# Biogod2020/Spatial-Clip

Hardware: AMD Instinct MI355X
Metric: tile-gene pairs/sec (train step) (higher is better)
Workload: dtype bf16

## Files before the change

spatial-clip_amd/csrc/sc_gemm8p.hip:

```cpp
#include "sc_gemm_common.h"
#include <stdlib.h>
#include <map>
#include <mutex>

namespace {

constexpr int BM = 256, BN = 256, BK = 64;
constexpr int HALF = 128 * 64 * 2;
constexpr int RING = 8 * HALF;
constexpr int EPI_BYTES = 8 * 64 * SC_EPI_LD * 4;
constexpr int LDS_BYTES = EPI_BYTES > RING ? EPI_BYTES : RING;

typedef const __attribute__((address_space(1))) void* gptr_t;
typedef __attribute__((address_space(3))) void* lptr_t;

SC_DEVICE void dma16(const void* src, char* lds_wave_base) {
    __builtin_amdgcn_global_load_lds((gptr_t)src, (lptr_t)lds_wave_base, 16, 0, 0);
}

template <int EPI, bool Q8 = false, bool LUT = false, int NI = 8>
SC_DEVICE void epilogue_bf16_lds(f32x4 (&acc)[NI][4], const GemmArgs& g, char* strip, int row0, int col0, int lane,
                                 const unsigned* lut = nullptr) {
    float amax_lane = 0.f;
    const float q8s = (Q8 && sc_epi_gelu_fwd(EPI) && g.q8) ? *g.q8_scale : 0.f;
    const int li = lane & 15, lg = lane >> 4;
    constexpr bool kBias = (EPI == SC_EPI_BF16_BIAS || sc_epi_gelu_fwd(EPI));
    f32x4 bj[4];
#pragma unroll
    for (int j = 0; j < 4; ++j) {
        bj[j] = (f32x4){0.f, 0.f, 0.f, 0.f};
        const int c = col0 + j * 16 + lg * 4;
        if (kBias && g.bias && c < g.N) bj[j] = *reinterpret_cast<const f32x4*>(g.bias + c);
    }
    bf16* C = reinterpret_cast<bf16*>(g.C);
    bf16* C2 = reinterpret_cast<bf16*>(g.C2);
    const int rr = lane >> 3, rc = lane & 7;
    const int gcol = col0 + rc * 8;
#pragma unroll
    for (int p = 0; p < NI / 2; ++p) {
#pragma unroll
        for (int ib = 0; ib < 2; ++ib) {
            const int r = ib * 16 + li;
#pragma unroll
            for (int j = 0; j < 4; ++j) {
// ... 49 lines not shown
                            for (int e = 0; e < 8; ++e) {
                                float hv, gv;
                                sc_act_both((float)x.h[e], g.act, hv, gv);
                                o[e] = (bf16)hv;
                                gd[e] = (bf16)gv;
                            }
                        }
                        *reinterpret_cast<bf16x8*>(C + (size_t)grow * g.ldc + gcol) = gd;
                    }
                    *reinterpret_cast<bf16x8*>(C2 + (size_t)grow * g.ldc2 + gcol) = o;
                    if (Q8 && g.q8) {
                        float r[8];
#pragma unroll
                        for (int e = 0; e < 8; ++e) { r[e] = (float)o[e]; amax_lane = fmaxf(amax_lane, fabsf(r[e])); }
                        *reinterpret_cast<u32x2*>(g.q8 + (size_t)grow * g.ldq8 + gcol) = sc_pack8_fp8(r, q8s);
                    }
                }
            }
        }
        __builtin_amdgcn_s_waitcnt(0xC07F);
        __builtin_amdgcn_wave_barrier();
    }
    if (Q8 && sc_epi_gelu_fwd(EPI) && g.q8) sc_amax_publish(amax_lane, g.q8_amax);
}

constexpr int slot(int D, int q) { return D * 4 * HALF + q * HALF; }

struct Stager {
    const bf16* src[4][2];
    int nt;
    int wave;
};

template <int D, int PH>
SC_DEVICE void phase(char* smem, const Stager& S, int t, const int (&a_off)[2], const int (&b_off)[2], bf16x8 (&a)[8],
                     bf16x8 (&b0)[4], bf16x8 (&b1)[4], f32x4 (&acc)[8][4]) {
    if (PH == 1) {
#pragma unroll
        for (int kk = 0; kk < 2; ++kk)
#pragma unroll
            for (int jj = 0; jj < 2; ++jj)
                b0[kk * 2 + jj] = *reinterpret_cast<const bf16x8*>(smem + slot(D, 1) + b_off[kk] + jj * 2048);
    }
    if (PH == 2) {
#pragma unroll
        for (int kk = 0; kk < 2; ++kk)
#pragma unroll
            for (int jj = 0; jj < 2; ++jj)
                b1[kk * 2 + jj] = *reinterpret_cast<const bf16x8*>(smem + slot(D, 2) + b_off[kk] + jj * 2048);
    }
    if (PH == 1 || PH == 3) {
        constexpr int sl = slot(D, PH == 1 ? 0 : 3);
#pragma unroll
        for (int kk = 0; kk < 2; ++kk)
#pragma unroll
            for (int ii = 0; ii < 4; ++ii)
                a[kk * 4 + ii] = *reinterpret_cast<const bf16x8*>(smem + sl + a_off[kk] + ii * 2048);
    }
    constexpr int q = (PH + 1) & 3;
    constexpr int DS = PH <= 2 ? (D ^ 1) : D;
    const int ts = t + (PH <= 2 ? 1 : 2);
    if (ts < S.nt) {
        dma16(S.src[q][0] + (size_t)ts * BK, smem + slot(DS, q) + S.wave * 1024);
        dma16(S.src[q][1] + (size_t)ts * BK, smem + slot(DS, q) + (8 + S.wave) * 1024);
        asm volatile("s_waitcnt vmcnt(8)" ::: "memory");
    } else {
        asm volatile("s_waitcnt vmcnt(0)" ::: "memory");
    }
    __builtin_amdgcn_sched_barrier(0);
    __builtin_amdgcn_s_barrier();
    __builtin_amdgcn_sched_barrier(0);
    constexpr int mi = PH >= 3 ? 1 : 0;
    constexpr int nj = (PH == 2 || PH == 3) ? 1 : 0;
    __builtin_amdgcn_s_setprio(1);
#pragma unroll
    for (int kk = 0; kk < 2; ++kk)
#pragma unroll
        for (int ii = 0; ii < 4; ++ii)
#pragma unroll
            for (int jj = 0; jj < 2; ++jj)
                acc[mi * 4 + ii][nj * 2 + jj] =
                    sc_mfma16(nj ? b1[kk * 2 + jj] : b0[kk * 2 + jj], a[kk * 4 + ii], acc[mi * 4 + ii][nj * 2 + jj]);
    __builtin_amdgcn_s_setprio(0);
    __builtin_amdgcn_sched_barrier(0);
    __builtin_amdgcn_s_barrier();
    __builtin_amdgcn_sched_barrier(0);
}

template <int D>
SC_DEVICE void ktile(char* smem, const Stager& S, int t, const int (&a_off)[2], const int (&b_off)[2], bf16x8 (&a)[8],
                     bf16x8 (&b0)[4], bf16x8 (&b1)[4], f32x4 (&acc)[8][4]) {
    phase<D, 1>(smem, S, t, a_off, b_off, a, b0, b1, acc);
    phase<D, 2>(smem, S, t, a_off, b_off, a, b0, b1, acc);
    phase<D, 3>(smem, S, t, a_off, b_off, a, b0, b1, acc);
    phase<D, 4>(smem, S, t, a_off, b_off, a, b0, b1, acc);
}

constexpr int HRING = 9 * HALF;
constexpr int hslot(int D, int q) { return (D * 3 + q) * HALF; }

struct HStager {
    const bf16* src[3][2];
    int nt;
    int wave;
};

template <int D, int PH>
SC_DEVICE void hphase(char* smem, const HStager& S, int t, const int (&a_off)[2], const int (&b_off)[2], bf16x8 (&a)[8],
                      bf16x8 (&b0)[4], bf16x8 (&b1)[4], f32x4 (&acc)[4][4]) {
    if (PH == 1) {
#pragma unroll
        for (int kk = 0; kk < 2; ++kk)
#pragma unroll
            for (int jj = 0; jj < 2; ++jj)
                b0[kk * 2 + jj] = *reinterpret_cast<const bf16x8*>(smem + hslot(D, 1) + b_off[kk] + jj * 2048);
#pragma unroll
        for (int kk = 0; kk < 2; ++kk)
#pragma unroll
            for (int ii = 0; ii < 4; ++ii)
                a[kk * 4 + ii] = *reinterpret_cast<const bf16x8*>(smem + hslot(D, 0) + a_off[kk] + ii * 2048);
    } else {
#pragma unroll
        for (int kk = 0; kk < 2; ++kk)
#pragma unroll
            for (int jj = 0; jj < 2; ++jj)
                b1[kk * 2 + jj] = *reinterpret_cast<const bf16x8*>(smem + hslot(D, 2) + b_off[kk] + jj * 2048);
    }
    constexpr int DS = (D + 2) % 3;
    const int ts = t + 2;
    if (ts < S.nt) {
        if (PH == 1) {
            dma16(S.src[0][0] + (size_t)ts * BK, smem + hslot(DS, 0) + S.wave * 1024);
            dma16(S.src[0][1] + (size_t)ts * BK, smem + hslot(DS, 0) + (8 + S.wave) * 1024);
            dma16(S.src[1][0] + (size_t)ts * BK, smem + hslot(DS, 1) + S.wave * 1024);
            dma16(S.src[1][1] + (size_t)ts * BK, smem + hslot(DS, 1) + (8 + S.wave) * 1024);
            asm volatile("s_waitcnt vmcnt(10)" ::: "memory");
        } else {
            dma16(S.src[2][0] + (size_t)ts * BK, smem + hslot(DS, 2) + S.wave * 1024);
            dma16(S.src[2][1] + (size_t)ts * BK, smem + hslot(DS, 2) + (8 + S.wave) * 1024);
            asm volatile("s_waitcnt vmcnt(8)" ::: "memory");
        }
    } else {
        asm volatile("s_waitcnt vmcnt(0)" ::: "memory");
    }
    __builtin_amdgcn_sched_barrier(0);
    __builtin_amdgcn_s_barrier();
    __builtin_amdgcn_sched_barrier(0);
    constexpr int nj = PH - 1;
    __builtin_amdgcn_s_setprio(1);
#pragma unroll
    for (int kk = 0; kk < 2; ++kk)
#pragma unroll
        for (int ii = 0; ii < 4; ++ii)
#pragma unroll
            for (int jj = 0; jj < 2; ++jj)
                acc[ii][nj * 2 + jj] = sc_mfma16(nj ? b1[kk * 2 + jj] : b0[kk * 2 + jj], a[kk * 4 + ii], acc[ii][nj * 2 + jj]);
    __builtin_amdgcn_s_setprio(0);
    __builtin_amdgcn_sched_barrier(0);
    __builtin_amdgcn_s_barrier();
    __builtin_amdgcn_sched_barrier(0);
}

template <int D>
SC_DEVICE void hktile(char* smem, const HStager& S, int t, const int (&a_off)[2], const int (&b_off)[2], bf16x8 (&a)[8],
                      bf16x8 (&b0)[4], bf16x8 (&b1)[4], f32x4 (&acc)[4][4]) {
    hphase<D, 1>(smem, S, t, a_off, b_off, a, b0, b1, acc);
    hphase<D, 2>(smem, S, t, a_off, b_off, a, b0, b1, acc);
}

template <int EPI>
SC_DEVICE void half_tile(const GemmArgs& g, char* smem, int mh, int n0) {
    const int t = threadIdx.x;
    const int lane = t & 63;
    const int wave = __builtin_amdgcn_readfirstlane(t >> 6);
    const int wr = wave >> 2, wc = wave & 3;
    const int li = lane & 15, lg = lane >> 4;

    HStager S;
    S.nt = g.K / BK;
    S.wave = wave;
#pragma unroll
    for (int p = 0; p < 2; ++p) {
        const int r = (p * 8 + wave) * 8 + (lane >> 3);
        const int lc = (lane & 7) ^ ((r >> 1) & 7);
        const int ga = min(mh + r, g.M - 1);
        S.src[0][p] = g.A + (size_t)ga * g.lda + lc * 8;
#pragma unroll
        for (int h = 0; h < 2; ++h) {
            const int gb = min(n0 + (r >> 5) * 64 + h * 32 + (r & 31), g.N - 1);
            S.src[1 + h][p] = g.B + (size_t)gb * g.ldb + lc * 8;
        }
    }
    int a_off[2], b_off[2];
#pragma unroll
    for (int kk = 0; kk < 2; ++kk) {
        const int coff = ((kk * 4 + lg) ^ ((li >> 1) & 7)) << 4;
        a_off[kk] = (wr * 64 + li) * 128 + coff;
        b_off[kk] = (wc * 32 + li) * 128 + coff;
    }
    f32x4 acc[4][4];
#pragma unroll
    for (int i = 0; i < 4; ++i)
#pragma unroll
        for (int j = 0; j < 4; ++j) acc[i][j] = (f32x4){0.f, 0.f, 0.f, 0.f};

#pragma unroll
    for (int s = 0; s < 6; ++s) {
        const int ts = s / 3, q = s % 3;
        if (ts < S.nt) {
            dma16(S.src[q][0] + (size_t)ts * BK, smem + hslot(ts, q) + wave * 1024);
            dma16(S.src[q][1] + (size_t)ts * BK, smem + hslot(ts, q) + (8 + wave) * 1024);
        }
    }
    if (S.nt > 1) asm volatile("s_waitcnt vmcnt(8)" ::: "memory");
    else asm volatile("s_waitcnt vmcnt(0)" ::: "memory");
    __builtin_amdgcn_sched_barrier(0);
    __builtin_amdgcn_s_barrier();
    if (wr == 1) __builtin_amdgcn_s_barrier();
    __builtin_amdgcn_sched_barrier(0);

    bf16x8 a[8], b0[4], b1[4];
    for (int kt = 0; kt < S.nt; kt += 3) {
        hktile<0>(smem, S, kt, a_off, b_off, a, b0, b1, acc);
        if (kt + 1 < S.nt) hktile<1>(smem, S, kt + 1, a_off, b_off, a, b0, b1, acc);
        if (kt + 2 < S.nt) hktile<2>(smem, S, kt + 2, a_off, b_off, a, b0, b1, acc);
    }
    if (wr == 0) __builtin_amdgcn_s_barrier();
    asm volatile("s_waitcnt vmcnt(0)" ::: "memory");
    __builtin_amdgcn_sched_barrier(0);

    const int row0 = mh + wr * 64, col0 = n0 + wc * 64;
    if (EPI == SC_EPI_GELU_GRAD_PAIR && g.gelu_lut != nullptr) {
        unsigned* lut = reinterpret_cast<unsigned*>(smem + 8 * 4096);
        for (int c = t; c < SC_GELU_LUT_N / 4; c += 512)
            reinterpret_cast<u32x4*>(lut)[c] = reinterpret_cast<const u32x4*>(g.gelu_lut)[c];
        __syncthreads();
        epilogue_bf16_lds<EPI, false, true>(acc, g, smem + wave * 4096, row0, col0, lane, lut);
    } else if (EPI == SC_EPI_BF16 || EPI == SC_EPI_BF16_BIAS || sc_epi_gelu_fwd(EPI)) {
        epilogue_bf16_lds<EPI>(acc, g, smem + wave * 4096, row0, col0, lane);
    } else {
        float* ep = reinterpret_cast<float*>(smem) + wave * 64 * SC_EPI_LD;
        EpiRegs<EPI> er;
        sc_epi_load<EPI>(er, row0, col0, lane, g, 64);
#pragma unroll
        for (int i = 0; i < 4; ++i)
#pragma unroll
            for (int j = 0; j < 4; ++j) sc_epi_put(ep, i, j, li, lg, acc[i][j]);
        __builtin_amdgcn_s_waitcnt(0xC07F);
        __builtin_amdgcn_wave_barrier();
        sc_epilogue_store<EPI>(ep, er, row0, col0, lane, g, 0, -1, 64);
    }
}

template <int EPI>
__global__ __launch_bounds__(512, 2) void gemm8p_kernel(const GemmArgs g) {
    extern __shared__ __attribute__((aligned(16))) char smem[];
    int idx, hh = -1;
    if (g.tail_first > 0) {
        const int b = (int)blockIdx.x - g.tail_first;
        if (b >= 0) {
            const int r = sc_xcd_remap(b, 2 * g.tail_rem);
            idx = g.tail_first + (r >> 1);
            hh = r & 1;
        } else {
            idx = sc_xcd_remap(blockIdx.x, g.tail_first);
        }
    } else {
        idx = sc_xcd_remap(blockIdx.x, gridDim.x);
    }
    int tn, tm, z;
    if (g.col_group > 0) {
        sc_tile_colgroup(idx, g, tm, tn);
        z = 0;
    } else {
        tn = idx % g.ntn;
        idx /= g.ntn;
// ... 14 lines not shown
    const int m0 = tm * BM, n0 = tn * BN;
    const int kbeg = z * g.k_per_split;
    const int kend = min(g.K, kbeg + g.k_per_split);

    Stager S;
    S.nt = (kend - kbeg) / BK;
    S.wave = wave;
#pragma unroll
    for (int p = 0; p < 2; ++p) {
        const int r = (p * 8 + wave) * 8 + (lane >> 3);
        const int lc = (lane & 7) ^ ((r >> 1) & 7);
#pragma unroll
        for (int h = 0; h < 2; ++h) {
            const int ga = min(m0 + (r >> 6) * 128 + h * 64 + (r & 63), g.M - 1);
            const int gb = min(n0 + (r >> 5) * 64 + h * 32 + (r & 31), g.N - 1);
            S.src[h ? 3 : 0][p] = g.A + (size_t)ga * g.lda + kbeg + lc * 8;
            S.src[h ? 2 : 1][p] = g.B + (size_t)gb * g.ldb + kbeg + lc * 8;
        }
    }
    int a_off[2], b_off[2];
#pragma unroll
    for (int kk = 0; kk < 2; ++kk) {
        const int coff = ((kk * 4 + lg) ^ ((li >> 1) & 7)) << 4;
        a_off[kk] = (wr * 64 + li) * 128 + coff;
        b_off[kk] = (wc * 32 + li) * 128 + coff;
    }

    f32x4 acc[8][4];
#pragma unroll
    for (int i = 0; i < 8; ++i)
#pragma unroll
        for (int j = 0; j < 4; ++j) acc[i][j] = (f32x4){0.f, 0.f, 0.f, 0.f};

#pragma unroll
    for (int s = 0; s < 6; ++s) {
        const int ts = s >> 2, q = s & 3;
        if (ts < S.nt) {
            dma16(S.src[q][0] + (size_t)ts * BK, smem + slot(ts & 1, q) + wave * 1024);
            dma16(S.src[q][1] + (size_t)ts * BK, smem + slot(ts & 1, q) + (8 + wave) * 1024);
        }
    }
    if (S.nt > 1) asm volatile("s_waitcnt vmcnt(8)" ::: "memory");
    else asm volatile("s_waitcnt vmcnt(0)" ::: "memory");
    __builtin_amdgcn_sched_barrier(0);
    __builtin_amdgcn_s_barrier();
    if (wr == 1) __builtin_amdgcn_s_barrier();
    __builtin_amdgcn_sched_barrier(0);

    bf16x8 a[8], b0[4], b1[4];
    for (int kt = 0; kt < S.nt; kt += 2) {
        ktile<0>(smem, S, kt, a_off, b_off, a, b0, b1, acc);
        if (kt + 1 < S.nt) ktile<1>(smem, S, kt + 1, a_off, b_off, a, b0, b1, acc);
    }
    if (wr == 0) __builtin_amdgcn_s_barrier();
    asm volatile("s_waitcnt vmcnt(0)" ::: "memory");
    __builtin_amdgcn_sched_barrier(0);

    if (EPI == SC_EPI_GELU_GRAD_PAIR && g.gelu_lut != nullptr) {
        unsigned* lut = reinterpret_cast<unsigned*>(smem + 8 * 4096);
        for (int c = t; c < SC_GELU_LUT_N / 4; c += 512)
            reinterpret_cast<u32x4*>(lut)[c] = reinterpret_cast<const u32x4*>(g.gelu_lut)[c];
        __syncthreads();
        epilogue_bf16_lds<EPI, false, true>(acc, g, smem + wave * 4096, m0 + wr * 128, n0 + wc * 64, lane, lut);
    } else if (EPI == SC_EPI_BF16 || EPI == SC_EPI_BF16_BIAS || sc_epi_gelu_fwd(EPI)) {
        epilogue_bf16_lds<EPI>(acc, g, smem + wave * 4096, m0 + wr * 128, n0 + wc * 64, lane);
    } else {
        const int mw = wr * 128;
        float* ep = reinterpret_cast<float*>(smem) + wave * 64 * SC_EPI_LD;
        EpiRegs<EPI> er;
        sc_epi_load<EPI>(er, m0 + mw, n0 + wc * 64, lane, g, 64);
#pragma unroll
        for (int h = 0; h < 2; ++h) {
#pragma unroll
            for (int i = 0; i < 4; ++i)
#pragma unroll
                for (int j = 0; j < 4; ++j) sc_epi_put(ep, i, j, li, lg, acc[h * 4 + i][j]);
            __builtin_amdgcn_s_waitcnt(0xC07F);
            __builtin_amdgcn_wave_barrier();
            sc_epilogue_store<EPI>(ep, er, m0 + mw + h * 64, n0 + wc * 64, lane, g, z, (h + 1 < 2) ? m0 + mw + 64 : -1, 64);
            __builtin_amdgcn_s_waitcnt(0xC07F);
            __builtin_amdgcn_wave_barrier();
        }
    }
}

__global__ void sc_gelu_lut_fill_kernel(unsigned* lut, int act) {
    const int i = blockIdx.x * blockDim.x + threadIdx.x;
    if (i >= SC_GELU_LUT_N) return;
    const unsigned bits = (unsigned)(SC_GELU_LUT_LO + i % SC_GELU_LUT_HALF) | (i >= SC_GELU_LUT_HALF ? 0x8000u : 0u);
    const float u = __uint_as_float(bits << 16);
    float hv, gv;
    sc_act_both(u, act, hv, gv);
    union { bf16 b; unsigned short s; } h, gq;
    h.b = (bf16)hv;
    gq.b = (bf16)gv;
    lut[i] = ((unsigned)gq.s << 16) | (unsigned)h.s;
}

template <int EPI>
int launch(const GemmArgs& g, int nblocks, hipStream_t st) {
    static bool attr_done = false;
    if (!attr_done) {
        (void)hipFuncSetAttribute(reinterpret_cast<const void*>(&gemm8p_kernel<EPI>),
                                  hipFuncAttributeMaxDynamicSharedMemorySize, LDS_BYTES > HRING ? LDS_BYTES : HRING);
        attr_done = true;
    }
    const int lds = (g.tail_first > 0 && HRING > LDS_BYTES) ? HRING : LDS_BYTES;
    gemm8p_kernel<EPI><<<nblocks, 512, lds, st>>>(g);
    SC_LAUNCH_CHECK();
    return 1;
}


enum { PW_STEADY = 0, PW_POSTEPI = 1, PW_DRAIN0 = 2 };

struct PStager {
    const bf16* src[4][2];
    long long koff;
    int sk;
    int stile;
    int nt, wave, total, stride;
};

SC_DEVICE void pstage_set_tile(PStager& S, const GemmArgs& g, int lane) {
    const int tn = S.stile % g.ntn, tm = S.stile / g.ntn;
    const int m0 = tm * BM, n0 = tn * BN;
#pragma unroll
    for (int p = 0; p < 2; ++p) {
        const int r = (p * 8 + S.wave) * 8 + (lane >> 3);
        const int lc = (lane & 7) ^ ((r >> 1) & 7);
#pragma unroll
        for (int h = 0; h < 2; ++h) {
            const int ga = min(m0 + (r >> 6) * 128 + h * 64 + (r & 63), g.M - 1);
            const int gb = min(n0 + (r >> 5) * 64 + h * 32 + (r & 31), g.N - 1);
            S.src[h ? 3 : 0][p] = g.A + (size_t)ga * g.lda + lc * 8;
            S.src[h ? 2 : 1][p] = g.B + (size_t)gb * g.ldb + lc * 8;
        }
    }
}
SC_DEVICE void pstage_advance(PStager& S, const GemmArgs& g, int lane) {
// ... 918 lines not shown
    static bool attr_done = false;
    if (!attr_done) {
        (void)hipFuncSetAttribute(reinterpret_cast<const void*>(&gemm8p_tn_f8_kernel), hipFuncAttributeMaxDynamicSharedMemorySize,
                                  LDS_BYTES);
        attr_done = true;
    }
    sc_gemm_note_path(SC_GEMM_PATH_FP8_TN, 0, 0, splitk, g.colsum ? SC_GEMM_COLSUM_FUSED : SC_GEMM_COLSUM_NONE);
    gemm8p_tn_f8_kernel<<<g.ntm * g.ntn * splitk, 512, LDS_BYTES, st>>>(g);
    SC_LAUNCH_CHECK();
    return 1;
}

static int sc_colgroup_default(int epi, const GemmArgs& g) {
    (void)epi; (void)g;
    return 0;
}

extern "C" int sc_debug_gemm_tail_rule(int T, int S, int* nfull, int* rem) {
    const int r = (S > 0 && T > S) ? T % S : 0;
    const bool split = r > 0 && 2 * r <= S;
    if (nfull) *nfull = split ? T - r : T;
    if (rem) *rem = split ? r : 0;
    return split ? 1 : 0;
}

static int sc_last_tail[2] = {-1, -1};
extern "C" int sc_debug_gemm_last_tail(int* nfull, int* rem, int reset) {
    if (nfull) *nfull = sc_last_tail[0];
    if (rem) *rem = sc_last_tail[1];
    if (reset) sc_last_tail[0] = sc_last_tail[1] = -1;
    return 0;
}

static int sc_last_path[6] = {SC_GEMM_PATH_NONE, 0, 0, 0, SC_GEMM_COLSUM_NONE, SC_GEMM_GROUP_NONE};
void sc_gemm_note_path(int path, int lut, int col_group, int splitk, int colsum) {
    sc_last_path[0] = path; sc_last_path[1] = lut; sc_last_path[2] = col_group; sc_last_path[3] = splitk;
    sc_last_path[4] = colsum; sc_last_path[5] = SC_GEMM_GROUP_NONE;
}
void sc_gemm_note_colsum(int colsum) { sc_last_path[4] = colsum; }
void sc_gemm_note_group(int group) { sc_last_path[5] = group; }
extern "C" int sc_debug_gemm_last_path(int* out, int n, int reset) {
    for (int i = 0; i < n && i < 6; ++i) out[i] = sc_last_path[i];
    if (reset) sc_gemm_note_path(SC_GEMM_PATH_NONE, 0, 0, 0, SC_GEMM_COLSUM_NONE);
    return 6;
}

static int sc_gemm_slots() {
    static int cus[64] = {};
    int dev = 0;
    if (hipGetDevice(&dev) != hipSuccess || dev < 0 || dev >= 64) return 0;
    if (cus[dev] == 0) {
        int n = 0;
        if (hipDeviceGetAttribute(&n, hipDeviceAttributeMultiprocessorCount, dev) != hipSuccess || n < 1) n = -1;
        cus[dev] = n;
    }
    return cus[dev] > 0 ? cus[dev] : 0;
}

static bool sc_tail_default(int epi, const GemmArgs& g) {
    (void)epi; (void)g;
    return true;
}

int sc_gemm8p_try(int mode, int epi, GemmArgs& g, int splitk_req, float* slabs, hipStream_t st) {
    if (g.M < 256 || g.N < 192 || (g.K % BK) != 0) return 0;
    if (mode == SC_GEMM_TN && (epi != SC_EPI_F32 || (g.M % 8) != 0 || (g.N % 8) != 0)) return 0;
    if ((long long)g.M * g.N < 256LL * 256 * 8) return 0;
    if (mode == SC_GEMM_NT && splitk_req <= 1) {
        static const int small_tiles = getenv("SC_GEMM_SMALL_TILES") ? atoi(getenv("SC_GEMM_SMALL_TILES")) : 100;
        if ((long long)g.M * g.N < 256LL * 256 * small_tiles) return 0;
    }
    g.ntm = (g.M + BM - 1) / BM;
    g.ntn = (g.N + BN - 1) / BN;
    const int ktiles = g.K / BK;
    int splitk = splitk_req < 1 ? 1 : splitk_req;
    if (epi != SC_EPI_F32 || slabs == nullptr) splitk = 1;
    if (splitk > ktiles) splitk = ktiles;
    int tiles_per = (ktiles + splitk - 1) / splitk;
    splitk = (ktiles + tiles_per - 1) / tiles_per;
    g.splitk = splitk;
    g.k_per_split = tiles_per * BK;
    g.slab_stride = 0;
    if (splitk > 1) {
        if (g.ldc != g.N) return 0;
        g.C = slabs;
        g.slab_stride = (long long)g.M * g.N;
    }
    const int nblocks = g.ntm * g.ntn * splitk;
    if (mode == SC_GEMM_TN) {
        sc_gemm_note_path(SC_GEMM_PATH_TN8P, 0, 0, splitk, g.colsum ? SC_GEMM_COLSUM_FUSED : SC_GEMM_COLSUM_NONE);
        return launch_tn(g, nblocks, st);
    }
// ... 13 lines not shown
    g.col_group = 0;
    if (splitk == 1 && g.ntn > 1) {
        int gc = sc_colgroup_default(epi, g);
        if (const char* sw = getenv("SC_GEMM_COLGROUP")) {
            for (const char* p = sw; *p;) {
                char* e = nullptr;
                const long ep = strtol(p, &e, 10);
                if (e == p || *e != ':') break;
                const long v = strtol(e + 1, &e, 10);
                if (ep == epi || ep == -1) gc = (int)v;
                p = (*e == ',') ? e + 1 : e;
                if (*e != ',') break;
            }
        }
        if (gc > 0 && gc < g.ntn) {
            g.col_group = gc;
            g.band_rows = (g.ntm + 7) / 8;
        }
    }
    g.tail_first = g.tail_rem = 0;
    int grid = nblocks;
    if (splitk == 1) {
        const char* sw = getenv("SC_GEMM_TAIL");
        const int slots = sw ? atoi(sw) : (sc_tail_default(epi, g) ? sc_gemm_slots() : 0);
        int nfull = 0, rem = 0;
        if (slots > 0 && sc_debug_gemm_tail_rule(nblocks, slots, &nfull, &rem)) {
            g.tail_first = nfull;
            g.tail_rem = rem;
            grid = nfull + 2 * rem;
        }
    }
    sc_last_tail[0] = g.tail_first > 0 ? g.tail_first : nblocks;
    sc_last_tail[1] = g.tail_rem;
    sc_gemm_note_path(SC_GEMM_PATH_NT8P, g.gelu_lut != nullptr, g.col_group, splitk, SC_GEMM_COLSUM_NONE);
    int rc = 0;
#define SC_CASE(EPI) \
    if (epi == EPI) rc = launch<EPI>(g, grid, st);
    SC_CASE(SC_EPI_BF16)
    SC_CASE(SC_EPI_BF16_BIAS)
    SC_CASE(SC_EPI_F32_BIAS_RES)
    SC_CASE(SC_EPI_GELU_PAIR)
    SC_CASE(SC_EPI_BF16_DGELU)
    SC_CASE(SC_EPI_F32)
    SC_CASE(SC_EPI_BF16_BIAS_RES)
    SC_CASE(SC_EPI_GELU_GRAD_PAIR)
    SC_CASE(SC_EPI_BF16_MUL_AUX)
#undef SC_CASE
    return rc;
}

const unsigned* sc_gelu_lut_device(hipStream_t st, int act) {
    static std::mutex mu;
    static std::map<int, unsigned*> all;
    int dev = 0;
    if (hipGetDevice(&dev) != hipSuccess) return nullptr;
    const int key = dev * 2 + (act ? 1 : 0);
    std::lock_guard<std::mutex> lock(mu);
    auto it = all.find(key);
    if (it != all.end()) return it->second;
    unsigned* p = nullptr;
    if (hipMalloc(reinterpret_cast<void**>(&p), SC_GELU_LUT_N * sizeof(unsigned)) != hipSuccess) p = nullptr;
    if (p) {
        sc_gelu_lut_fill_kernel<<<(SC_GELU_LUT_N + 255) / 256, 256, 0, st>>>(p, act ? 1 : 0);
        if (hipGetLastError() != hipSuccess || hipStreamSynchronize(st) != hipSuccess) {
            (void)hipFree(p);
            p = nullptr;
        }
// ... 5 lines not shown
```

spatial-clip_amd/csrc/sc_gemm_common.h:

```cpp
#pragma once
#include "sc_common.h"
#include "sc_kernels.h"

struct GemmArgs {
    const bf16* A;
    const bf16* B;
    int M, N, K;
    int lda, ldb;
    void* C;
    int ldc;
    void* C2;
    int ldc2;
    const float* bias;
    const float* res;
    int ldres;
    const bf16* aux;
    int ldaux;
    int splitk;
    int k_per_split;
    long long slab_stride;
    int ntm, ntn;
    int tile_offset;
    float* colsum;
    const float* a_scale = nullptr;
    const float* b_scale = nullptr;
    unsigned char* q8 = nullptr;
    long long ldq8 = 0;
    const float* q8_scale = nullptr;
    float* q8_amax = nullptr;
    int a_scale_scalar = 0;
    const unsigned* gelu_lut = nullptr;
    int act = 0;
    int col_group = 0;
    int band_rows = 0;
    int tail_first = 0;
    int tail_rem = 0;
};

SC_DEVICE void sc_tile_colgroup(int idx, const GemmArgs& g, int& tm, int& tn) {
    const int band_tiles = g.band_rows * g.ntn;
    const int band = idx / band_tiles;
    const int r = idx - band * band_tiles;
    const int row0 = band * g.band_rows;
    const int rows = min(g.band_rows, g.ntm - row0);
    const int nfg = g.ntn / g.col_group;
    const int full = rows * g.col_group * nfg;
    if (r < full) {
        const int gsz = rows * g.col_group;
        const int grp = r / gsz, rr = r - grp * gsz;
        tm = row0 + rr / g.col_group;
        tn = grp * g.col_group + rr % g.col_group;
    } else {
        const int rem = g.ntn - nfg * g.col_group, r2 = r - full;
        tm = row0 + r2 / rem;
        tn = nfg * g.col_group + r2 % rem;
    }
}

constexpr int SC_GELU_LUT_LO = 107 << 7;
constexpr int SC_GELU_LUT_HALF = 25 * 128;
constexpr int SC_GELU_LUT_N = 2 * SC_GELU_LUT_HALF;
const unsigned* sc_gelu_lut_device(hipStream_t st, int act = 0);

constexpr int SC_EPI_LD = 68;

SC_DEVICE void sc_gelu_qe(float x, float& q, float& e) {
    const float y = fabsf(x) * 0.84932180028801904f;
    const float t = __builtin_amdgcn_rcpf(__builtin_fmaf(0.2727374808792225f, y, 1.0f));
    e = __builtin_amdgcn_exp2f(-(y * y));
// ... 50 lines not shown
constexpr bool sc_epi_gelu_fwd(int e) { return e == SC_EPI_GELU_PAIR || e == SC_EPI_GELU_GRAD_PAIR; }
constexpr bool sc_epi_aux_mul(int e) { return e == SC_EPI_BF16_DGELU || e == SC_EPI_BF16_MUL_AUX; }

SC_DEVICE u32x2 sc_pack8_fp8(const float (&v)[8], float s) {
    float c[8];
#pragma unroll
    for (int k = 0; k < 8; ++k) c[k] = fminf(fmaxf(v[k] * s, -448.f), 448.f);
    int w0 = __builtin_amdgcn_cvt_pk_fp8_f32(c[0], c[1], 0, false);
    w0 = __builtin_amdgcn_cvt_pk_fp8_f32(c[2], c[3], w0, true);
    int w1 = __builtin_amdgcn_cvt_pk_fp8_f32(c[4], c[5], 0, false);
    w1 = __builtin_amdgcn_cvt_pk_fp8_f32(c[6], c[7], w1, true);
    return (u32x2){(unsigned)w0, (unsigned)w1};
}
SC_DEVICE void sc_amax_publish(float amax_lane, float* slots) {
    float a = amax_lane;
#pragma unroll
    for (int off = 32; off > 0; off >>= 1) a = fmaxf(a, __shfl_xor(a, off, 64));
    if ((threadIdx.x & 63) == 0 && a > 0.f)
        atomicMax(reinterpret_cast<unsigned*>(slots) + (blockIdx.x & 63), __float_as_uint(a));
}

SC_DEVICE void sc_epi_put(float* ep, int row16, int col16, int li, int lg, f32x4 acc) {
    *reinterpret_cast<f32x4*>(ep + (row16 * 16 + li) * SC_EPI_LD + col16 * 16 + lg * 4) = acc;
}

template <int EPI>
struct EpiRegs {
    static constexpr bool kRes = (EPI == SC_EPI_F32_BIAS_RES);
    static constexpr bool kAux = (sc_epi_aux_mul(EPI) || EPI == SC_EPI_BF16_BIAS_RES);
    f32x4 r[kRes ? 16 : 1];
    bf16x8 a[kAux ? 8 : 1];
};

template <int EPI>
SC_DEVICE void sc_epi_load(EpiRegs<EPI>& e, int gm0, int gn0, int lane, const GemmArgs& g, int mrows = 64) {
    const int mlim = min(g.M, gm0 + mrows);
    if (EPI == SC_EPI_F32_BIAS_RES) {
        const int gn = gn0 + (lane & 15) * 4;
#pragma unroll
        for (int ps = 0; ps < 16; ++ps) {
            const int gm = gm0 + ps * 4 + (lane >> 4);
            e.r[ps] = (f32x4){0.f, 0.f, 0.f, 0.f};
            if (g.res && gm < mlim && gn < g.N) e.r[ps] = *reinterpret_cast<const f32x4*>(g.res + (size_t)gm * g.ldres + gn);
        }
    }
    if (sc_epi_aux_mul(EPI)) {
        const int gn = gn0 + (lane & 7) * 8;
#pragma unroll
        for (int ps = 0; ps < 8; ++ps) {
            const int gm = gm0 + ps * 8 + (lane >> 3);
            if (gm < mlim && gn < g.N) e.a[ps] = *reinterpret_cast<const bf16x8*>(g.aux + (size_t)gm * g.ldaux + gn);
        }
    }
    if (EPI == SC_EPI_BF16_BIAS_RES) {
        const int gn = gn0 + (lane & 7) * 8;
        const bf16* res = reinterpret_cast<const bf16*>(g.res);
#pragma unroll
        for (int ps = 0; ps < 8; ++ps) {
            const int gm = gm0 + ps * 8 + (lane >> 3);
#pragma unroll
            for (int k = 0; k < 8; ++k) e.a[ps][k] = (bf16)0.0f;
            if (res && gm < mlim && gn < g.N) e.a[ps] = *reinterpret_cast<const bf16x8*>(res + (size_t)gm * g.ldres + gn);
        }
    }
}

template <int EPI, bool Q8 = false>
SC_DEVICE void sc_epilogue_store(const float* ep, EpiRegs<EPI>& e, int gm0, int gn0, int lane, const GemmArgs& g, int z,
                                 int next_gm0 = -1, int mrows = 64, int hi_col_skip = 0, float* amax_lane = nullptr) {
    const int mlim = min(g.M, gm0 + mrows);
    if (EPI == SC_EPI_F32 || EPI == SC_EPI_F32_BIAS_RES) {
        float* C = reinterpret_cast<float*>(g.C) + (size_t)z * g.slab_stride;
        const int col = (lane & 15) * 4;
        const int gn = gn0 + col + ((col >> 5) ? hi_col_skip : 0);
        f32x4 bv = (f32x4){0.f, 0.f, 0.f, 0.f};
        if (EPI == SC_EPI_F32_BIAS_RES && g.bias && gn < g.N) bv = *reinterpret_cast<const f32x4*>(g.bias + gn);
#pragma unroll
        for (int ps = 0; ps < 16; ++ps) {
            const int row = ps * 4 + (lane >> 4);
            const int gm = gm0 + row;
            f32x4 v = *reinterpret_cast<const f32x4*>(ep + row * SC_EPI_LD + col);
            if (EPI == SC_EPI_F32_BIAS_RES) {
                v += bv + e.r[ps];
                if (next_gm0 >= 0) {
                    const int gm2 = next_gm0 + row;
                    e.r[ps] = (f32x4){0.f, 0.f, 0.f, 0.f};
                    if (g.res && gm2 < g.M && gn < g.N)
                        e.r[ps] = *reinterpret_cast<const f32x4*>(g.res + (size_t)gm2 * g.ldres + gn);
                }
            }
            if (gm < mlim && gn < g.N) *reinterpret_cast<f32x4*>(C + (size_t)gm * g.ldc + gn) = v;
// ... 49 lines not shown
                if (EPI != SC_EPI_GELU_GRAD_PAIR) *reinterpret_cast<bf16x8*>(C + (size_t)gm * g.ldc + gn) = o;
                if (Q8 && sc_epi_aux_mul(EPI) && g.q8) {
                    float r[8];
#pragma unroll
                    for (int k = 0; k < 8; ++k) { r[k] = (float)o[k]; *amax_lane = fmaxf(*amax_lane, fabsf(r[k])); }
                    *reinterpret_cast<u32x2*>(g.q8 + (size_t)gm * g.ldq8 + gn) = sc_pack8_fp8(r, *g.q8_scale);
                }
                if (EPI == SC_EPI_GELU_PAIR) {
                    bf16x8 h;
#pragma unroll
                    for (int k = 0; k < 8; ++k) h[k] = (bf16)sc_act((float)o[k], g.act);
                    *reinterpret_cast<bf16x8*>(reinterpret_cast<bf16*>(g.C2) + (size_t)gm * g.ldc2 + gn) = h;
                }
                if (EPI == SC_EPI_GELU_GRAD_PAIR) {
                    bf16x8 h, gd;
#pragma unroll
                    for (int k = 0; k < 8; ++k) {
                        float hv, gv;
                        sc_act_both((float)o[k], g.act, hv, gv);
                        h[k] = (bf16)hv;
                        gd[k] = (bf16)gv;
                    }
                    *reinterpret_cast<bf16x8*>(C + (size_t)gm * g.ldc + gn) = gd;
                    *reinterpret_cast<bf16x8*>(reinterpret_cast<bf16*>(g.C2) + (size_t)gm * g.ldc2 + gn) = h;
                }
            }
        }
    }
}

void sc_gemm_note_path(int path, int lut, int col_group, int splitk, int colsum);
void sc_gemm_note_colsum(int colsum);
void sc_gemm_note_group(int group);

int sc_gemm256_try(int mode, int epi, GemmArgs& g, int splitk_req, float* slabs, float* c_final, hipStream_t st);
int sc_gemm8p_try(int mode, int epi, GemmArgs& g, int splitk_req, float* slabs, hipStream_t st);
int sc_gemm8p_tn_group_plan(const GemmArgs* g, int n, int splitk_req, int* splitk_out, int* k_per_split);
int sc_gemm8p_tn_group_launch(const GemmArgs* g, int n, hipStream_t st);
int sc_gemm8p_tn_fp8(GemmArgs& g, int splitk_req, float* slabs, hipStream_t st);
int sc_gemm8p_fp8(int epi, GemmArgs& g, hipStream_t st);
```

spatial-clip_amd/ops.py:

```python
from __future__ import annotations

import collections
import ctypes
from typing import Optional

import torch

from . import _lib
from ._lib import check

NT, TN = 0, 1
(EPI_BF16, EPI_BF16_BIAS, EPI_F32_BIAS_RES, EPI_GELU_PAIR, EPI_BF16_DGELU, EPI_F32, EPI_BF16_BIAS_RES, EPI_GELU_GRAD_PAIR,
 EPI_BF16_MUL_AUX, EPI_QGELU_PAIR, EPI_BF16_DQGELU, EPI_QGELU_GRAD_PAIR) = range(12)


def act_epilogues(quick_gelu: bool):
    if quick_gelu:
        return EPI_QGELU_PAIR, EPI_QGELU_GRAD_PAIR, EPI_BF16_DQGELU
    return EPI_GELU_PAIR, EPI_GELU_GRAD_PAIR, EPI_BF16_DGELU


def _stream() -> int:
    return torch.cuda.current_stream().cuda_stream

# ... 164 lines not shown
    check(fn(ctypes.byref(f), ctypes.byref(b)), "sc_debug_attn_last_path")
    return (ATTN_FWD_PATHS[f.value] if f.value >= 0 else "none", ATTN_BWD_PATHS[b.value] if b.value >= 0 else "none")


def attn_plan(B: int, L: int, H: int, dh: int, causal: bool = False, q_rows: int = 0):
    fn = getattr(_lib.lib(), "sc_debug_attn_plan")
    fn.restype, fn.argtypes = ctypes.c_int, [ctypes.c_int] * 6 + [ctypes.POINTER(ctypes.c_int)] * 2
    f, b = ctypes.c_int(-1), ctypes.c_int(-1)
    check(fn(B, L, H, dh, int(causal), q_rows, ctypes.byref(f), ctypes.byref(b)), "sc_debug_attn_plan")
    return ATTN_FWD_PATHS[f.value], ATTN_BWD_PATHS[b.value]


def gemm_tail_rule(T: int, S: int):
    fn = getattr(_lib.lib(), "sc_debug_gemm_tail_rule")
    fn.restype, fn.argtypes = ctypes.c_int, [ctypes.c_int] * 2 + [ctypes.POINTER(ctypes.c_int)] * 2
    nfull, rem = ctypes.c_int(-1), ctypes.c_int(-1)
    split = fn(T, S, ctypes.byref(nfull), ctypes.byref(rem))
    assert bool(split) == (rem.value > 0)
    return nfull.value, rem.value


def gemm_last_tail(reset: bool = False):
    fn = getattr(_lib.lib(), "sc_debug_gemm_last_tail")
    fn.restype, fn.argtypes = ctypes.c_int, [ctypes.POINTER(ctypes.c_int)] * 2 + [ctypes.c_int]
    nfull, rem = ctypes.c_int(-1), ctypes.c_int(-1)
    fn(ctypes.byref(nfull), ctypes.byref(rem), int(reset))
    return nfull.value, rem.value


GEMM_PATHS = ("nt128", "nt128_ktail", "tn128", "nt8p", "nt8p_persistent", "tn8p", "tn8p_group", "nt256", "tn256", "fp8_nt",
              "fp8_tn")
GEMM_COLSUMS = ("none", "fused", "separate")
GEMM_GROUPS = ("none", "one_launch", "per_problem")
GemmPath = collections.namedtuple("GemmPath", "path lut col_group splitk colsum group")


def gemm_last_path(reset: bool = False) -> GemmPath:
    fn = getattr(_lib.lib(), "sc_debug_gemm_last_path")
    fn.restype, fn.argtypes = ctypes.c_int, [ctypes.POINTER(ctypes.c_int), ctypes.c_int, ctypes.c_int]
    out = (ctypes.c_int * 6)()
    assert fn(out, 6, int(reset)) == 6
    return GemmPath(GEMM_PATHS[out[0]] if out[0] >= 0 else "none", bool(out[1]), out[2], out[3], GEMM_COLSUMS[out[4]],
                    GEMM_GROUPS[out[5]])


def _t8_args(t8, rows: int, d: int, what: str):
    buf, scale, amax = t8
    if buf.dtype != torch.uint8 or not buf.is_cuda or buf.stride(-1) != 1 or buf.shape[0] < rows or buf.shape[1] < d:
        raise TypeError(f"{what}: t8 buffer must be a device uint8 matrix of at least [{rows}, {d}]")
    _req(scale, torch.float32, "t8 scale"); _req(amax, torch.float32, "t8 amax")
    if scale.numel() != 1 or amax.numel() != 64:
        raise ValueError(f"{what}: t8 needs a one-element scale and 64 amax slots")
    return buf.data_ptr(), buf.stride(0), scale.data_ptr(), amax.data_ptr()


def layernorm_fwd(x, gamma, beta, y, mean, rstd, rows: int, d: int, ldx: Optional[int] = None,
                  ldy: Optional[int] = None, eps: float = 1e-5, q8: Optional[torch.Tensor] = None,
                  q8_scale_inv: Optional[torch.Tensor] = None, t8=None):
    _req(y, torch.bfloat16, "y")
    if q8 is not None:
        if q8.dtype != torch.uint8 or not q8.is_cuda or q8.stride(-1) != 1:
            raise TypeError("layernorm_fwd: q8 must be a device uint8 matrix")
        _req(q8_scale_inv, torch.float32, "q8_scale_inv")
    if t8 is not None and (x.dtype != torch.bfloat16 or q8 is None):
        raise _lib.SpatialClipHipError("layernorm_fwd: the per-tensor e4m3 copy exists for bf16 rows with the per-row copy (q8)")
    if x.dtype == torch.bfloat16 and t8 is not None:
        tp, tld, tsc, tam = _t8_args(t8, rows, d, "layernorm_fwd")
        check(_lib.lib().sc_layernorm_fwd_x16_t8(x.data_ptr(), ldx if ldx is not None else d, gamma.data_ptr(), beta.data_ptr(),
                                                 y.data_ptr(), ldy if ldy is not None else d, q8.data_ptr(), q8.stride(0),
                                                 q8_scale_inv.data_ptr(), tp, tld, tsc, tam, _ptr(mean), _ptr(rstd), rows, d, eps,
                                                 _stream()), "sc_layernorm_fwd_x16_t8")
        return y
    if x.dtype == torch.bfloat16:
        _req(x, torch.bfloat16, "x")
        check(_lib.lib().sc_layernorm_fwd_x16(x.data_ptr(), ldx if ldx is not None else d, gamma.data_ptr(), beta.data_ptr(),
                                              y.data_ptr(), ldy if ldy is not None else d, _ptr(q8),
# ... 534 lines not shown
```

Baseline: 8191.

## Prefetch epilogue aux/residual rows and GELU LUT into LDS during main loop

During the last K-tile of the 8-phase GEMM, the first few rows of the epilogue's aux or residual operand are now fetched into spare LDS above the ring with async global-to-LDS loads. The epilogue reads those rows from LDS and loads only the remainder from global memory. For the GELU-grad epilogue, the lookup table is staged into LDS at kernel start instead of being copied synchronously after the main loop. The aim is to hide epilogue load latency behind the MFMA loop, at the cost of requesting 160 KiB of LDS, which may lower occupancy. Both paths are on by default and can be disabled with an environment variable.

```diff
diff --git a/spatial-clip_amd/csrc/sc_gemm8p.hip b/spatial-clip_amd/csrc/sc_gemm8p.hip
--- a/spatial-clip_amd/csrc/sc_gemm8p.hip
+++ b/spatial-clip_amd/csrc/sc_gemm8p.hip
@@ -10,6 +10,10 @@
 constexpr int RING = 8 * HALF;
 constexpr int EPI_BYTES = 8 * 64 * SC_EPI_LD * 4;
 constexpr int LDS_BYTES = EPI_BYTES > RING ? EPI_BYTES : RING;
+constexpr int LUT_BYTES = SC_GELU_LUT_N * 4;
+constexpr int HRING = 9 * HALF;
+constexpr int LDS_ALL = 160 * 1024;
+static_assert(LUT_BYTES % 1024 == 0 && RING + LUT_BYTES <= LDS_ALL, "the table is copied in 1-KiB wave pieces");
 
 typedef const __attribute__((address_space(1))) void* gptr_t;
 typedef __attribute__((address_space(3))) void* lptr_t;
@@ -125,9 +129,59 @@
     int wave;
 };
 
-template <int D, int PH>
+constexpr int PRE_NP_FULL = 3, PRE_NP_HALF = 2;
+static_assert(EPI_BYTES + 8 * PRE_NP_FULL * 1024 <= LDS_ALL && EPI_BYTES >= RING, "full tile: pieces above ring and fp32 staging");
+static_assert(HRING + 8 * PRE_NP_HALF * 1024 <= LDS_ALL && HRING >= EPI_BYTES, "half tile: pieces above its ring and the staging");
+template <int EPI>
+struct Preload {
+    static constexpr bool kOn = EpiRegs<EPI>::kAux;
+    bool on;
+    char* dst;
+    int gm0, gn0, lane;
+};
+template <int EPI, int NP>
+SC_DEVICE void drain_wait(const Preload<EPI>& P, const GemmArgs& g, bool last, bool issue) {
+    if constexpr (Preload<EPI>::kOn) {
+        if (P.on && last) {
+            if (issue) {
+                const bf16* src = EPI == SC_EPI_BF16_BIAS_RES ? reinterpret_cast<const bf16*>(g.res) : g.aux;
+                const int ld = EPI == SC_EPI_BF16_BIAS_RES ? g.ldres : g.ldaux;
+                const int gn = min(P.gn0 + (P.lane & 7) * 8, g.N - 8);
+#pragma unroll
+                for (int ps = 0; ps < NP; ++ps) {
+                    const int gm = min(P.gm0 + ps * 8 + (P.lane >> 3), g.M - 1);
+                    dma16(src + (size_t)gm * ld + gn, P.dst + ps * 1024);
+                }
+            }
+            asm volatile("s_waitcnt vmcnt(%0)" ::"n"(NP) : "memory");
+            return;
+        }
+    }
+    asm volatile("s_waitcnt vmcnt(0)" ::: "memory");
+}
+template <int EPI, int NP>
+SC_DEVICE void epi_load_first(EpiRegs<EPI>& er, const Preload<EPI>& P, const GemmArgs& g) {
+    if constexpr (Preload<EPI>::kOn) {
+#ifdef SC_DIAG_EPI_NO_INPUT
+#pragma unroll
+        for (int ps = 0; ps < 8; ++ps)
+#pragma unroll
+            for (int k = 0; k < 8; ++k) er.a[ps][k] = (bf16)1.0f;
+        return;
+#endif
+        if (P.on) {
+#pragma unroll
+            for (int ps = 0; ps < NP; ++ps) er.a[ps] = *reinterpret_cast<const bf16x8*>(P.dst + ps * 1024 + P.lane * 16);
+            sc_epi_load<EPI, NP>(er, P.gm0, P.gn0, P.lane, g, 64);
+            return;
+        }
+    }
+    sc_epi_load<EPI>(er, P.gm0, P.gn0, P.lane, g, 64);
+}
+
+template <int D, int PH, int EPI>
 SC_DEVICE void phase(char* smem, const Stager& S, int t, const int (&a_off)[2], const int (&b_off)[2], bf16x8 (&a)[8],
-                     bf16x8 (&b0)[4], bf16x8 (&b1)[4], f32x4 (&acc)[8][4]) {
+                     bf16x8 (&b0)[4], bf16x8 (&b1)[4], f32x4 (&acc)[8][4], Preload<EPI>& P, const GemmArgs& g) {
     if (PH == 1) {
 #pragma unroll
         for (int kk = 0; kk < 2; ++kk)
@@ -158,7 +212,7 @@
         dma16(S.src[q][1] + (size_t)ts * BK, smem + slot(DS, q) + (8 + S.wave) * 1024);
         asm volatile("s_waitcnt vmcnt(8)" ::: "memory");
     } else {
-        asm volatile("s_waitcnt vmcnt(0)" ::: "memory");
+        drain_wait<EPI, PRE_NP_FULL>(P, g, t == S.nt - 1, PH == 1);
     }
     __builtin_amdgcn_sched_barrier(0);
     __builtin_amdgcn_s_barrier();
@@ -180,16 +234,15 @@
     __builtin_amdgcn_sched_barrier(0);
 }
 
-template <int D>
+template <int D, int EPI>
 SC_DEVICE void ktile(char* smem, const Stager& S, int t, const int (&a_off)[2], const int (&b_off)[2], bf16x8 (&a)[8],
-                     bf16x8 (&b0)[4], bf16x8 (&b1)[4], f32x4 (&acc)[8][4]) {
-    phase<D, 1>(smem, S, t, a_off, b_off, a, b0, b1, acc);
-    phase<D, 2>(smem, S, t, a_off, b_off, a, b0, b1, acc);
-    phase<D, 3>(smem, S, t, a_off, b_off, a, b0, b1, acc);
-    phase<D, 4>(smem, S, t, a_off, b_off, a, b0, b1, acc);
-}
-
-constexpr int HRING = 9 * HALF;
+                     bf16x8 (&b0)[4], bf16x8 (&b1)[4], f32x4 (&acc)[8][4], Preload<EPI>& P, const GemmArgs& g) {
+    phase<D, 1, EPI>(smem, S, t, a_off, b_off, a, b0, b1, acc, P, g);
+    phase<D, 2, EPI>(smem, S, t, a_off, b_off, a, b0, b1, acc, P, g);
+    phase<D, 3, EPI>(smem, S, t, a_off, b_off, a, b0, b1, acc, P, g);
+    phase<D, 4, EPI>(smem, S, t, a_off, b_off, a, b0, b1, acc, P, g);
+}
+
 constexpr int hslot(int D, int q) { return (D * 3 + q) * HALF; }
 
 struct HStager {
@@ -198,9 +251,9 @@
     int wave;
 };
 
-template <int D, int PH>
+template <int D, int PH, int EPI>
 SC_DEVICE void hphase(char* smem, const HStager& S, int t, const int (&a_off)[2], const int (&b_off)[2], bf16x8 (&a)[8],
-                      bf16x8 (&b0)[4], bf16x8 (&b1)[4], f32x4 (&acc)[4][4]) {
+                      bf16x8 (&b0)[4], bf16x8 (&b1)[4], f32x4 (&acc)[4][4], Preload<EPI>& P, const GemmArgs& g) {
     if (PH == 1) {
 #pragma unroll
         for (int kk = 0; kk < 2; ++kk)
@@ -234,7 +287,7 @@
             asm volatile("s_waitcnt vmcnt(8)" ::: "memory");
         }
     } else {
-        asm volatile("s_waitcnt vmcnt(0)" ::: "memory");
+        drain_wait<EPI, PRE_NP_HALF>(P, g, t == S.nt - 1, PH == 1);
     }
     __builtin_amdgcn_sched_barrier(0);
     __builtin_amdgcn_s_barrier();
@@ -254,11 +307,11 @@
     __builtin_amdgcn_sched_barrier(0);
 }
 
-template <int D>
+template <int D, int EPI>
 SC_DEVICE void hktile(char* smem, const HStager& S, int t, const int (&a_off)[2], const int (&b_off)[2], bf16x8 (&a)[8],
-                      bf16x8 (&b0)[4], bf16x8 (&b1)[4], f32x4 (&acc)[4][4]) {
-    hphase<D, 1>(smem, S, t, a_off, b_off, a, b0, b1, acc);
-    hphase<D, 2>(smem, S, t, a_off, b_off, a, b0, b1, acc);
+                      bf16x8 (&b0)[4], bf16x8 (&b1)[4], f32x4 (&acc)[4][4], Preload<EPI>& P, const GemmArgs& g) {
+    hphase<D, 1, EPI>(smem, S, t, a_off, b_off, a, b0, b1, acc, P, g);
+    hphase<D, 2, EPI>(smem, S, t, a_off, b_off, a, b0, b1, acc, P, g);
 }
 
 template <int EPI>
@@ -312,17 +365,22 @@
     if (wr == 1) __builtin_amdgcn_s_barrier();
     __builtin_amdgcn_sched_barrier(0);
 
+    const int row0 = mh + wr * 64, col0 = n0 + wc * 64;
+    Preload<EPI> P;
+    P.on = g.epi_preload != 0;
+    P.dst = smem + HRING + wave * (PRE_NP_HALF * 1024);
+    P.gm0 = row0; P.gn0 = col0; P.lane = lane;
+
     bf16x8 a[8], b0[4], b1[4];
     for (int kt = 0; kt < S.nt; kt += 3) {
-        hktile<0>(smem, S, kt, a_off, b_off, a, b0, b1, acc);
-        if (kt + 1 < S.nt) hktile<1>(smem, S, kt + 1, a_off, b_off, a, b0, b1, acc);
-        if (kt + 2 < S.nt) hktile<2>(smem, S, kt + 2, a_off, b_off, a, b0, b1, acc);
+        hktile<0, EPI>(smem, S, kt, a_off, b_off, a, b0, b1, acc, P, g);
+        if (kt + 1 < S.nt) hktile<1, EPI>(smem, S, kt + 1, a_off, b_off, a, b0, b1, acc, P, g);
+        if (kt + 2 < S.nt) hktile<2, EPI>(smem, S, kt + 2, a_off, b_off, a, b0, b1, acc, P, g);
     }
     if (wr == 0) __builtin_amdgcn_s_barrier();
     asm volatile("s_waitcnt vmcnt(0)" ::: "memory");
     __builtin_amdgcn_sched_barrier(0);
 
-    const int row0 = mh + wr * 64, col0 = n0 + wc * 64;
     if (EPI == SC_EPI_GELU_GRAD_PAIR && g.gelu_lut != nullptr) {
         unsigned* lut = reinterpret_cast<unsigned*>(smem + 8 * 4096);
         for (int c = t; c < SC_GELU_LUT_N / 4; c += 512)
@@ -334,7 +392,7 @@
     } else {
         float* ep = reinterpret_cast<float*>(smem) + wave * 64 * SC_EPI_LD;
         EpiRegs<EPI> er;
-        sc_epi_load<EPI>(er, row0, col0, lane, g, 64);
+        epi_load_first<EPI, PRE_NP_HALF>(er, P, g);
 #pragma unroll
         for (int i = 0; i < 4; ++i)
 #pragma unroll
@@ -415,6 +473,10 @@
 #pragma unroll
         for (int j = 0; j < 4; ++j) acc[i][j] = (f32x4){0.f, 0.f, 0.f, 0.f};
 
+    if (EPI == SC_EPI_GELU_GRAD_PAIR && g.lut_staged) {
+        for (int c = wave; c < LUT_BYTES / 1024; c += 8)
+            dma16(reinterpret_cast<const char*>(g.gelu_lut) + c * 1024 + lane * 16, smem + RING + c * 1024);
+    }
 #pragma unroll
     for (int s = 0; s < 6; ++s) {
         const int ts = s >> 2, q = s & 3;
@@ -430,20 +492,29 @@
     if (wr == 1) __builtin_amdgcn_s_barrier();
     __builtin_amdgcn_sched_barrier(0);
 
+    Preload<EPI> P;
+    P.on = g.epi_preload != 0;
+    P.dst = smem + EPI_BYTES + wave * (PRE_NP_FULL * 1024);
+    P.gm0 = m0 + wr * 128; P.gn0 = n0 + wc * 64; P.lane = lane;
+
     bf16x8 a[8], b0[4], b1[4];
     for (int kt = 0; kt < S.nt; kt += 2) {
-        ktile<0>(smem, S, kt, a_off, b_off, a, b0, b1, acc);
-        if (kt + 1 < S.nt) ktile<1>(smem, S, kt + 1, a_off, b_off, a, b0, b1, acc);
+        ktile<0, EPI>(smem, S, kt, a_off, b_off, a, b0, b1, acc, P, g);
+        if (kt + 1 < S.nt) ktile<1, EPI>(smem, S, kt + 1, a_off, b_off, a, b0, b1, acc, P, g);
     }
     if (wr == 0) __builtin_amdgcn_s_barrier();
     asm volatile("s_waitcnt vmcnt(0)" ::: "memory");
     __builtin_amdgcn_sched_barrier(0);
 
     if (EPI == SC_EPI_GELU_GRAD_PAIR && g.gelu_lut != nullptr) {
-        unsigned* lut = reinterpret_cast<unsigned*>(smem + 8 * 4096);
-        for (int c = t; c < SC_GELU_LUT_N / 4; c += 512)
-            reinterpret_cast<u32x4*>(lut)[c] = reinterpret_cast<const u32x4*>(g.gelu_lut)[c];
-        __syncthreads();
+        unsigned* lut = reinterpret_cast<unsigned*>(smem + (g.lut_staged ? RING : 8 * 4096));
+        if (!g.lut_staged) {
+#ifndef SC_DIAG_EPI_NO_INPUT
+            for (int c = t; c < SC_GELU_LUT_N / 4; c += 512)
+                reinterpret_cast<u32x4*>(lut)[c] = reinterpret_cast<const u32x4*>(g.gelu_lut)[c];
+#endif
+            __syncthreads();
+        }
         epilogue_bf16_lds<EPI, false, true>(acc, g, smem + wave * 4096, m0 + wr * 128, n0 + wc * 64, lane, lut);
     } else if (EPI == SC_EPI_BF16 || EPI == SC_EPI_BF16_BIAS || sc_epi_gelu_fwd(EPI)) {
         epilogue_bf16_lds<EPI>(acc, g, smem + wave * 4096, m0 + wr * 128, n0 + wc * 64, lane);
@@ -451,7 +522,7 @@
         const int mw = wr * 128;
         float* ep = reinterpret_cast<float*>(smem) + wave * 64 * SC_EPI_LD;
         EpiRegs<EPI> er;
-        sc_epi_load<EPI>(er, m0 + mw, n0 + wc * 64, lane, g, 64);
+        epi_load_first<EPI, PRE_NP_FULL>(er, P, g);
 #pragma unroll
         for (int h = 0; h < 2; ++h) {
 #pragma unroll
@@ -485,10 +556,10 @@
     static bool attr_done = false;
     if (!attr_done) {
         (void)hipFuncSetAttribute(reinterpret_cast<const void*>(&gemm8p_kernel<EPI>),
-                                  hipFuncAttributeMaxDynamicSharedMemorySize, LDS_BYTES > HRING ? LDS_BYTES : HRING);
+                                  hipFuncAttributeMaxDynamicSharedMemorySize, LDS_ALL);
         attr_done = true;
     }
-    const int lds = (g.tail_first > 0 && HRING > LDS_BYTES) ? HRING : LDS_BYTES;
+    const int lds = (g.lut_staged || g.epi_preload) ? LDS_ALL : (g.tail_first > 0 && HRING > LDS_BYTES) ? HRING : LDS_BYTES;
     gemm8p_kernel<EPI><<<nblocks, 512, lds, st>>>(g);
     SC_LAUNCH_CHECK();
     return 1;
@@ -1473,17 +1544,18 @@
     return 0;
 }
 
-static int sc_last_path[6] = {SC_GEMM_PATH_NONE, 0, 0, 0, SC_GEMM_COLSUM_NONE, SC_GEMM_GROUP_NONE};
+static int sc_last_path[8] = {SC_GEMM_PATH_NONE, 0, 0, 0, SC_GEMM_COLSUM_NONE, SC_GEMM_GROUP_NONE, 0, 0};
 void sc_gemm_note_path(int path, int lut, int col_group, int splitk, int colsum) {
     sc_last_path[0] = path; sc_last_path[1] = lut; sc_last_path[2] = col_group; sc_last_path[3] = splitk;
-    sc_last_path[4] = colsum; sc_last_path[5] = SC_GEMM_GROUP_NONE;
-}
+    sc_last_path[4] = colsum; sc_last_path[5] = SC_GEMM_GROUP_NONE; sc_last_path[6] = sc_last_path[7] = 0;
+}
+void sc_gemm_note_preload(int loads, int lut_staged) { sc_last_path[6] = loads; sc_last_path[7] = lut_staged; }
 void sc_gemm_note_colsum(int colsum) { sc_last_path[4] = colsum; }
 void sc_gemm_note_group(int group) { sc_last_path[5] = group; }
 extern "C" int sc_debug_gemm_last_path(int* out, int n, int reset) {
-    for (int i = 0; i < n && i < 6; ++i) out[i] = sc_last_path[i];
+    for (int i = 0; i < n && i < 8; ++i) out[i] = sc_last_path[i];
     if (reset) sc_gemm_note_path(SC_GEMM_PATH_NONE, 0, 0, 0, SC_GEMM_COLSUM_NONE);
-    return 6;
+    return 8;
 }
 
 static int sc_gemm_slots() {
@@ -1499,6 +1571,11 @@
 }
 
 static bool sc_tail_default(int epi, const GemmArgs& g) {
+    (void)epi; (void)g;
+    return true;
+}
+
+static bool sc_epi_preload_default(int epi, const GemmArgs& g) {
     (void)epi; (void)g;
     return true;
 }
@@ -1578,7 +1655,15 @@
     }
     sc_last_tail[0] = g.tail_first > 0 ? g.tail_first : nblocks;
     sc_last_tail[1] = g.tail_rem;
+    g.epi_preload = g.lut_staged = 0;
+    {
+        const char* sw = getenv("SC_GEMM_EPI_PRELOAD");
+        const bool on = sw ? sw[0] != '0' : sc_epi_preload_default(epi, g);
+        if (on && (sc_epi_aux_mul(epi) || (epi == SC_EPI_BF16_BIAS_RES && g.res != nullptr))) g.epi_preload = 1;
+        if (on && epi == SC_EPI_GELU_GRAD_PAIR && g.gelu_lut != nullptr) g.lut_staged = 1;
+    }
     sc_gemm_note_path(SC_GEMM_PATH_NT8P, g.gelu_lut != nullptr, g.col_group, splitk, SC_GEMM_COLSUM_NONE);
+    sc_gemm_note_preload(g.epi_preload ? PRE_NP_FULL : 0, g.lut_staged);
     int rc = 0;
 #define SC_CASE(EPI) \
     if (epi == EPI) rc = launch<EPI>(g, grid, st);
diff --git a/spatial-clip_amd/csrc/sc_gemm_common.h b/spatial-clip_amd/csrc/sc_gemm_common.h
--- a/spatial-clip_amd/csrc/sc_gemm_common.h
+++ b/spatial-clip_amd/csrc/sc_gemm_common.h
@@ -35,6 +35,8 @@
     int band_rows = 0;
     int tail_first = 0;
     int tail_rem = 0;
+    int epi_preload = 0;
+    int lut_staged = 0;
 };
 
 SC_DEVICE void sc_tile_colgroup(int idx, const GemmArgs& g, int& tm, int& tn) {
@@ -151,7 +153,7 @@
     bf16x8 a[kAux ? 8 : 1];
 };
 
-template <int EPI>
+template <int EPI, int PS0 = 0>
 SC_DEVICE void sc_epi_load(EpiRegs<EPI>& e, int gm0, int gn0, int lane, const GemmArgs& g, int mrows = 64) {
     const int mlim = min(g.M, gm0 + mrows);
     if (EPI == SC_EPI_F32_BIAS_RES) {
@@ -166,7 +168,7 @@
     if (sc_epi_aux_mul(EPI)) {
         const int gn = gn0 + (lane & 7) * 8;
 #pragma unroll
-        for (int ps = 0; ps < 8; ++ps) {
+        for (int ps = PS0; ps < 8; ++ps) {
             const int gm = gm0 + ps * 8 + (lane >> 3);
             if (gm < mlim && gn < g.N) e.a[ps] = *reinterpret_cast<const bf16x8*>(g.aux + (size_t)gm * g.ldaux + gn);
         }
@@ -175,7 +177,7 @@
         const int gn = gn0 + (lane & 7) * 8;
         const bf16* res = reinterpret_cast<const bf16*>(g.res);
 #pragma unroll
-        for (int ps = 0; ps < 8; ++ps) {
+        for (int ps = PS0; ps < 8; ++ps) {
             const int gm = gm0 + ps * 8 + (lane >> 3);
 #pragma unroll
             for (int k = 0; k < 8; ++k) e.a[ps][k] = (bf16)0.0f;
@@ -291,6 +293,7 @@
 void sc_gemm_note_path(int path, int lut, int col_group, int splitk, int colsum);
 void sc_gemm_note_colsum(int colsum);
 void sc_gemm_note_group(int group);
+void sc_gemm_note_preload(int loads, int lut_staged);
 
 int sc_gemm256_try(int mode, int epi, GemmArgs& g, int splitk_req, float* slabs, float* c_final, hipStream_t st);
 int sc_gemm8p_try(int mode, int epi, GemmArgs& g, int splitk_req, float* slabs, hipStream_t st);
diff --git a/spatial-clip_amd/ops.py b/spatial-clip_amd/ops.py
--- a/spatial-clip_amd/ops.py
+++ b/spatial-clip_amd/ops.py
@@ -220,16 +220,16 @@
               "fp8_tn")
 GEMM_COLSUMS = ("none", "fused", "separate")
 GEMM_GROUPS = ("none", "one_launch", "per_problem")
-GemmPath = collections.namedtuple("GemmPath", "path lut col_group splitk colsum group")
+GemmPath = collections.namedtuple("GemmPath", "path lut col_group splitk colsum group preload lut_staged", defaults=(0, False))
 
 
 def gemm_last_path(reset: bool = False) -> GemmPath:
     fn = getattr(_lib.lib(), "sc_debug_gemm_last_path")
     fn.restype, fn.argtypes = ctypes.c_int, [ctypes.POINTER(ctypes.c_int), ctypes.c_int, ctypes.c_int]
-    out = (ctypes.c_int * 6)()
-    assert fn(out, 6, int(reset)) == 6
+    out = (ctypes.c_int * 8)()
+    assert fn(out, 8, int(reset)) == 8
     return GemmPath(GEMM_PATHS[out[0]] if out[0] >= 0 else "none", bool(out[1]), out[2], out[3], GEMM_COLSUMS[out[4]],
-                    GEMM_GROUPS[out[5]])
+                    GEMM_GROUPS[out[5]], out[6], bool(out[7]))
 
 
 def _t8_args(t8, rows: int, d: int, what: str):
```

After: 8244, median of 6. No clear change (+0.6%).
